# mindspore-lab/minddiffusion

Measured on AMD Instinct MI355X. Metric: 512x512 txt2img latents/sec (50-step DDIM), higher is better.
Workload: dtype f16; 1 GPU; SDv2 txt2img 512x512 (64x64 latent), 50-step DDIM, CFG 9.0, batch 1 per GPU (BASELINE.json configs[1]); synthetic seeded weights + synthetic text conditioning; global_batch=1, parallelism=batch-shard x1, hip_graph=True, rccl_world_size=1, broadcast_bytes=0, ddim_steps=50, unet_batch_per_gpu=2, sampler=ddim, cfg_dup_prefix=False

## Files before the change

minddiffusion_amd/_lib.py:

```python
import ctypes
import os

_HERE = os.path.dirname(os.path.abspath(__file__))
LIB_PATH = os.environ.get("MDX_LIBRARY") or os.path.join(_HERE, "libmdx.so")

c_void_p = ctypes.c_void_p
c_int = ctypes.c_int
c_uint = ctypes.c_uint
c_long = ctypes.c_long
c_float = ctypes.c_float
c_size_t = ctypes.c_size_t


class MdxError(RuntimeError):
    pass


class GemmDesc(ctypes.Structure):
    _fields_ = [
        ("a", c_void_p), ("a2", c_void_p), ("c1", c_int), ("c2", c_int),
        ("w", c_void_p), ("bias", c_void_p), ("rowbias", c_void_p), ("rowbias_ld", c_int),
        ("residual", c_void_p), ("residual_ld", c_int),
        ("out", c_void_p), ("out_ld", c_int),
        ("B", c_int), ("H", c_int), ("W", c_int), ("N", c_int),
# ... 136 lines not shown
                                       c_int, c_int, c_int, c_void_p]),
    "mdx_mask_feather_f32": (c_int, [c_void_p, c_void_p, c_int, c_void_p, c_int, c_int, c_int, c_void_p]),
    "mdx_inpaint_composite_f32": (c_int, [c_void_p, c_void_p, c_void_p, c_int, c_void_p, c_void_p, c_int, c_int, c_int,
                                          c_int, c_void_p]),
    "mdx_philox_u32": (c_int, [c_void_p, c_uint, c_uint, c_void_p, c_int, c_long, c_void_p]),
    "mdx_randn_f32": (c_int, [c_void_p, c_uint, c_uint, c_float, c_float, c_void_p, c_int, c_long, c_void_p]),
    "mdx_randn_slots_f32": (c_int, [c_void_p, c_uint, c_uint, c_float, c_float, c_void_p, c_void_p, c_void_p, c_int, c_int,
                                    c_long, c_void_p]),
    "mdx_slot_blend_f32": (c_int, [c_void_p, c_void_p, c_void_p, c_void_p, c_uint, c_uint, c_void_p, c_void_p, c_void_p,
                                   c_void_p, c_int, c_int, c_int, c_int, c_int, c_void_p]),
    "mdx_softmax_rows_f16": (c_int, [c_void_p, c_long, c_int, c_int, c_float, c_void_p]),
    "mdx_probe_mfma_32x32x16_f16": (c_int, [c_void_p, c_void_p, c_void_p, c_void_p]),
    "mdx_probe_mfma_16x16x32_f16": (c_int, [c_void_p, c_void_p, c_void_p, c_void_p]),
    "mdx_probe_gemm_trace": (c_int, [c_void_p, c_size_t]),
    "mdx_probe_valu_rate": (c_int, [c_int, c_int, c_int, c_void_p, c_void_p]),
    "mdx_probe_mix_rate": (c_int, [c_int, c_int, c_int, c_void_p, c_void_p]),
    "mdx_probe_l2_stream": (c_int, [c_void_p, c_size_t, ctypes.c_uint, c_int, c_int, c_int, c_int, c_void_p, c_void_p]),
    "mdx_probe_dma_stream": (c_int, [c_void_p, c_size_t, c_int, c_int, c_int, c_int, c_int, c_int, c_void_p, c_void_p]),
}

_lib = None
_ENV_OPTIONS = {
    "MDX_GEMM_TUNED": ("gemm_tuned", int), "MDX_GEMM_BM": ("gemm_bm", int), "MDX_GEMM_BN": ("gemm_bn", int),
    "MDX_GEMM_CFG": ("gemm_ring", lambda v: int(v.split(",")[-1])), "MDX_GEMM_HALO": ("gemm_halo", int),
    "MDX_GEMM_HALO8": ("gemm_halo8", int), "MDX_GEMM_SPLITK_FIXUP_MAX": ("gemm_splitk_fixup_max", int),
    "MDX_GEMM_SPREAD": ("gemm_spread", int), "MDX_HALO_NSB": ("halo_nsb", int), "MDX_GN_MIN_BLOCKS": ("gn_min_blocks", int),
    "MDX_GN_FUSED": ("gn_fused", int), "MDX_GN_COL_CHUNKS": ("gn_col_chunks", int),
    "MDX_GEMM_CONV8P": ("gemm_conv8p", int), "MDX_GEMM_CONV8P_MIN_M": ("gemm_conv8p_min_m", int),
    "MDX_GEMM_SUBPIXEL_MIN_TILES": ("gemm_subpixel_min_tiles", int), "MDX_GEMM_CONV8P_VAR": ("gemm_conv8p_var", int),
    "MDX_ATTN8": ("attn8", int), "MDX_ATTN8_MIN_BLOCKS": ("attn8_min_blocks", int),
    "MDX_GN_WIDE_ROWS": ("gn_wide_rows", int), "MDX_GN_BOOST_MB": ("gn_boost_mb", int), "MDX_ATTN_OCC3": ("attn_occ3", int), "MDX_ATTN_KV_SPLIT": ("attn_kv_split", int),
    "MDX_ATTN_FAST_STAGE": ("attn_fast_stage", int), "MDX_GN_PREFETCH": ("gn_prefetch", int), "MDX_GEMM_LN_PREFETCH": ("gemm_ln_prefetch", int),
    "MDX_GEMM_DENSE_ISSUE": ("gemm_dense_issue", int), "MDX_GEMM_LEAN_DENSE": ("gemm_lean_dense", int),
    "MDX_ATTN_PIPE": ("attn_pipe", int),
}


def load():
    global _lib
    if _lib is not None:
        return _lib
    if not os.path.exists(LIB_PATH):
        raise MdxError(
            f"{LIB_PATH} not found: the HIP extension is required (no CPU fallback). "
            "Build it with `python -c 'import __graft_entry__ as g; g.build()'` or `make -C minddiffusion_amd/csrc`.")
    import torch
    lib = ctypes.CDLL(LIB_PATH)
    for name, (res, args) in SIGNATURES.items():
        fn = getattr(lib, name)
        fn.restype = res
        fn.argtypes = args
    for env, (name, conv) in _ENV_OPTIONS.items():
        if env in os.environ:
            rc = lib.mdx_set_option(name.encode(), conv(os.environ[env]))
            if rc != 0:
                raise MdxError(f"{env}: {lib.mdx_last_error().decode()}")
    _lib = lib
    return lib


def check(rc, what):
    if rc != 0:
        msg = load().mdx_last_error()
        raise MdxError(f"{what} failed (rc={rc}): {msg.decode() if msg else ''}")
```

minddiffusion_amd/csrc/gemm.hip:

```cpp
#include "mdx_common.h"
#include "gemm_internal.h"

#include <algorithm>
#include <type_traits>

namespace {


template <int BM, int BN, int BK, int NS, bool SWAP, bool FASTK, int NW, bool GNA = false, bool EXT = false>
__global__ __launch_bounds__(NW * 64, NW == 4 ? 2 : 1) void gemm_kernel(const GemmParams p) {
    mdx_kernarg_touch<sizeof(GemmParams)>();
    constexpr int WROWS = BM / (NW / 2);
    constexpr int TM = WROWS / 32;
    constexpr int TN = BN / 64;
    static_assert(TM >= 1, "tile too short for this many waves");
    constexpr int ROWB = BK * 2;
    constexpr int CPRW = BK / 8;
    constexpr int RPI = 64 / CPRW;
    constexpr int RP256 = 256 / ROWB;
    constexpr int KS = BK / 16;
    constexpr int A_BYTES = BM * ROWB;
    constexpr int B_BYTES = BN * ROWB;
    constexpr int STAGE = A_BYTES + B_BYTES;
    constexpr int AJ = BM / RPI / NW;
    constexpr int BJ = BN / RPI / NW;
    static_assert(AJ >= 1 && BJ >= 1, "tile too small for this many loader waves");
    extern __shared__ __attribute__((aligned(16))) char smem[];

    const int tid = threadIdx.x;
    const int lane = tid & 63;
    const int wave = __builtin_amdgcn_readfirstlane(tid >> 6);
    const int wm = wave >> 1, wn = wave & 1;
    const int hi = lane >> 5;
    const int l31 = lane & 31;

    const int ntiles = p.tiles_m * p.tiles_n;
    const int tile_id = p.spread ? (int)(blockIdx.x % (unsigned)ntiles) : (blockIdx.x & 7) * p.tiles_per_xcd + (blockIdx.x >> 3);
// ... 291 lines not shown
            using I2 = std::integral_constant<int, 2>;
            using I3 = std::integral_constant<int, 3>;
            rdfrag(I0{}, 0); rdfrag(I1{}, 1); rdfrag(I2{}, 2); rdfrag(I3{}, 3);
            __builtin_amdgcn_sched_barrier(0);
            mfmas(I0{}); mfmas(I1{}); mfmas(I2{}); mfmas(I3{});
        } else {
            rdfrag(I0{}, 0);
            __builtin_amdgcn_sched_barrier(0);
#pragma unroll
            for (int ks = 0; ks < KS; ks += 2) {
                rdfrag(I1{}, ks + 1);
                __builtin_amdgcn_sched_barrier(0);
                mfmas(I0{});
                __builtin_amdgcn_sched_barrier(0);
                if (ks + 2 < KS) {
                    rdfrag(I0{}, ks + 2);
                    __builtin_amdgcn_sched_barrier(0);
                }
                mfmas(I1{});
                __builtin_amdgcn_sched_barrier(0);
            }
        }
        rd = (rd + 1 == NS) ? 0 : rd + 1;
        wr = (wr + 1 == NS) ? 0 : wr + 1;
    }

    __syncthreads();
    trace_mark(p, 3);
    if constexpr (SWAP) asm volatile("" ::"v"(touch_ln), "v"(touch_s));
    gemm_epilogue<BM, BN, SWAP, NW, LinearRows, 0, 0, EXT>(p, acc, smem, LinearRows{m0}, n0, split, bpre, tile_m, tile_id);
    trace_mark(p, 4);
}

template <int BM, int BN, int NSB, bool SWAP, int PW, bool BDIR = false, bool W4 = false>
__global__ __launch_bounds__(BM * 2, BM == 128 ? 2 : 1) void conv3x3_halo_kernel(const GemmParams p) {
    static_assert(PW == 16 || (PW == 8 && BM == 128), "patch width 16, or 8 with two-sample tiles");
    static_assert(!W4 || (BDIR && BM == 128 && BN == 128 && !SWAP), "W4: weight-streaming 128 x 128 tiles with slab output");
    constexpr int NW = BM / 32;
    constexpr int PH = BM / 16;
    constexpr int HWD = PW + 2;
    constexpr int WROWS = W4 ? BM : BM / (NW / 2);
    constexpr int TM = WROWS / 32;
    constexpr int TN = W4 ? 1 : BN / 64;
    constexpr int HROWS = PW == 16 ? (PH + 2) * 18 : (BM / 64) * 100;
    constexpr int HINST = (HROWS + 7) / 8;
    constexpr int HALO_BYTES = HINST * 1024;
    constexpr int HJ = (HINST + NW - 1) / NW;
    constexpr int B_BYTES = BN * 128;
    constexpr int BJ = BN / 8 / NW;
    static_assert(BJ >= 1, "weight tile too small for this many loader waves");
    extern __shared__ __attribute__((aligned(16))) char smem[];
    mdx_kernarg_touch<sizeof(GemmParams)>();

    const int tid = threadIdx.x;
    const int lane = tid & 63;
    const int wave = __builtin_amdgcn_readfirstlane(tid >> 6);
    const int wm = W4 ? 0 : wave >> 1, wn = W4 ? wave : wave & 1;
    const int hi = lane >> 5;
    const int l31 = lane & 31;

    const int ntiles = p.tiles_m * p.tiles_n;
    const int tile_id = p.spread ? (int)(blockIdx.x % (unsigned)ntiles) : (blockIdx.x & 7) * p.tiles_per_xcd + (blockIdx.x >> 3);
    if (tile_id >= ntiles) return;
    int tile_m, tile_n;
    if (p.n_fastest) {
        tile_m = tile_id / p.tiles_n;
        tile_n = tile_id - tile_m * p.tiles_n;
    } else {
        tile_n = tile_id / p.tiles_m;
        tile_m = tile_id - tile_n * p.tiles_m;
    }
    trace_mark(p, 0);
    const int n0 = tile_n * BN;
    const int pw = PW == 16 ? p.W >> 4 : 1, ph = PW == 16 ? p.H / PH : 1;
    const int pb = PW == 16 ? tile_m / (ph * pw) : tile_m * (BM / 64);
    const int prem = PW == 16 ? tile_m - pb * (ph * pw) : 0;
    const int py0 = (prem / pw) * PH, px0 = (prem % pw) * 16;
    const int split = p.spread ? (int)(blockIdx.x / (unsigned)ntiles) : (int)blockIdx.y;
    const int kt_begin = split * p.ktiles_per_split;
    const int kt_end = min(p.ktiles, kt_begin + p.ktiles_per_split);
    const int nt = kt_end - kt_begin;
    const int c_begin = kt_begin / 9, c_end = kt_end / 9;

    const __amdgpu_buffer_rsrc_t rs_a = make_rsrc(p.a, p.a_bytes);
    const __amdgpu_buffer_rsrc_t rs_w = make_rsrc(p.w, p.w_bytes);

    const int lrow = lane >> 3, lchk = lane & 7;
    unsigned hal_off[HJ];
    const unsigned row_bytes = (unsigned)p.cin * 2;
#pragma unroll
    for (int q = 0; q < HJ; ++q) {
        const int hp = (wave * HJ + q) * 8 + lrow;
        if constexpr (PW == 16) {
            const int hr = hp / 18, hc = hp - hr * 18;
            const int y = py0 - 1 + hr, x = px0 - 1 + hc;
            const bool ok = hp < HROWS && y >= 0 && y < p.H && x >= 0 && x < p.W;
            hal_off[q] = ok ? (unsigned)((pb * p.H + y) * p.W + x) * row_bytes + (unsigned)((lchk ^ ((hc >> 1) & 7)) * 16)
                            : MDX_OOB;
        } else {
            const int sm = hp / 100, r = hp - sm * 100;
            const int hr = r / 10, hc = r - hr * 10;
            const int y = hr - 1, x = hc - 1;
            const bool ok = hp < HROWS && pb + sm < p.B && y >= 0 && y < 8 && x >= 0 && x < 8;
            const int key = ((hc >> 1) & 3) | ((hr & 1) << 2);
            hal_off[q] = ok ? (unsigned)(((pb + sm) * 8 + y) * 8 + x) * row_bytes + (unsigned)((lchk ^ key) * 16) : MDX_OOB;
        }
    }
    unsigned b_off[BJ];
#pragma unroll
    for (int j = 0; j < BJ; ++j) {
        const int row = (wave * BJ + j) * 8 + lrow;
        const int panel = (n0 >> 6) + (row >> 6);
        b_off[j] = (unsigned)(((size_t)panel * p.kt64) * 8192 + ((row & 63) * 8 + lchk) * 16);
    }
    auto dma_halo = [&](int q, int chunk, int hb) {
        if (wave * HJ + q >= HINST) return;
        const unsigned off = hal_off[q] == MDX_OOB ? MDX_OOB : hal_off[q] + (unsigned)chunk * 128u;
        dma16(rs_a, smem + hb * HALO_BYTES + (wave * HJ + q) * 1024, off);
    };
    auto dma_b = [&](int kt, int stage) {
        char* sb = smem + 2 * HALO_BYTES + stage * B_BYTES;
#pragma unroll
        for (int j = 0; j < BJ; ++j) dma16s(rs_w, sb + (wave * BJ + j) * 1024, b_off[j], (unsigned)kt * 8192u);
    };

    f32x16 acc[TM][TN];
#pragma unroll
    for (int i = 0; i < TM; ++i)
#pragma unroll
        for (int j = 0; j < TN; ++j)
#pragma unroll
            for (int r = 0; r < 16; ++r) acc[i][j][r] = 0.f;

    int hp0[TM];
#pragma unroll
    for (int i = 0; i < TM; ++i) {
        const int q = wm * WROWS + i * 32 + l31;
        hp0[i] = PW == 16 ? (q >> 4) * 18 + (q & 15) : (q >> 6) * 100 + ((q >> 3) & 7) * 10 + (q & 7);
    }
    const int swz_b = (l31 >> 1) & 7;
    const int b_row_off = 2 * HALO_BYTES + (wn * (BN / 2) + l31) * 128;

    float bpre[16];
    gemm_bias_prefetch<BN, SWAP, NW>(p, n0, bpre);

    if constexpr (BDIR) {
        constexpr int PFB = 12;
        const unsigned kpieces = (unsigned)p.kt64 * 4u;
        unsigned pbase[TN];
#pragma unroll
        for (int j = 0; j < TN; ++j)
            pbase[j] = (unsigned)((n0 + (W4 ? wn * 32 : wn * (BN / 2) + j * 32)) >> 5) * kpieces + (unsigned)kt_begin * 4u;
        const unsigned voffw = (unsigned)lane * 16u;
#pragma unroll
        for (int q = 0; q < HJ; ++q) dma_halo(q, c_begin, 0);
        u32x4 ring[TN][PFB];
#pragma unroll
        for (int q = 0; q < PFB; ++q)
#pragma unroll
            for (int j = 0; j < TN; ++j) ring[j][q] = __builtin_amdgcn_raw_buffer_load_b128(rs_w, voffw, (pbase[j] + q) * 1024u, 0);
        trace_mark(p, 1);
        unsigned step = 0;
        for (int c = c_begin; c < c_end; ++c) {
            const int hb = (c - c_begin) & 1;
            asm volatile("s_waitcnt vmcnt(%0)" ::"n"(PFB * TN) : "memory");
            __builtin_amdgcn_s_barrier();
            if (c + 1 < c_end) {
#pragma unroll
                for (int q = 0; q < HJ; ++q) dma_halo(q, c + 1, hb ^ 1);
            }
#pragma unroll
            for (int tap = 0; tap < 9; ++tap) {
                const int ky = tap / 3, kx = tap - ky * 3;
                const int dq = ky * HWD + kx;
                int a_row[TM], a_key[TM];
#pragma unroll
                for (int i = 0; i < TM; ++i) {
                    a_row[i] = hb * HALO_BYTES + (hp0[i] + dq) * 128;
                    if constexpr (PW == 16)
                        a_key[i] = ((((l31 & 15) + kx) >> 1) & 7) << 4;
                    else
                        a_key[i] = (((((l31 & 7) + kx) >> 1) & 3) | ((((l31 >> 3) + ky) & 1) << 2)) << 4;
                }
#pragma unroll
                for (int s = 0; s < 4; ++s) {
                    f16x8 af[TM];
#pragma unroll
                    for (int i = 0; i < TM; ++i)
                        af[i] = *reinterpret_cast<const f16x8*>(smem + a_row[i] + (((2 * s + hi) << 4) ^ a_key[i]));
                    constexpr int dummy = 0;
                    (void)dummy;
                    const int rp = (tap * 4 + s) % PFB;
#pragma unroll
                    for (int j = 0; j < TN; ++j) {
                        const f16x8 b = __builtin_bit_cast(f16x8, ring[j][rp]);
                        ring[j][rp] = __builtin_amdgcn_raw_buffer_load_b128(rs_w, voffw, (pbase[j] + step + (unsigned)(tap * 4 + s) + PFB) * 1024u, 0);
#pragma unroll
                        for (int i = 0; i < TM; ++i) {
                            if constexpr (SWAP)
                                acc[i][j] = __builtin_amdgcn_mfma_f32_32x32x16_f16(b, af[i], acc[i][j], 0, 0, 0);
                            else
                                acc[i][j] = __builtin_amdgcn_mfma_f32_32x32x16_f16(af[i], b, acc[i][j], 0, 0, 0);
                        }
                    }
                    __builtin_amdgcn_sched_barrier(0);
                }
            }
            step += 36;
        }
        asm volatile("s_waitcnt vmcnt(0)" ::: "memory");
        __syncthreads();
        trace_mark(p, 3);
        if constexpr (W4) {
            float* wsz = p.ws + (size_t)split * p.M * p.N;
            const int n = n0 + wn * 32 + l31;
#pragma unroll
            for (int i = 0; i < TM; ++i)
#pragma unroll
                for (int r = 0; r < 16; ++r) {
                    const int row = i * 32 + (r & 3) + 8 * (r >> 2) + 4 * hi;
                    int m;
                    if constexpr (PW == 16)
                        m = (pb * p.H + py0) * p.W + px0 + (row >> 4) * p.W + (row & 15);
                    else
                        m = tile_m * BM + row;
                    if (m < p.M && n < p.N) wsz[(size_t)m * p.N + n] = acc[i][0][r];
                }
            trace_mark(p, 4);
            return;
        } else {
            if constexpr (PW == 16)
                gemm_epilogue<BM, BN, SWAP, NW, PatchRows, 0, 2>(p, acc, smem, PatchRows{(pb * p.H + py0) * p.W + px0, p.W, pb}, n0,
                                                                          split, bpre, tile_m, tile_id);
            else
                gemm_epilogue<BM, BN, SWAP, NW>(p, acc, smem, LinearRows{tile_m * BM}, n0, split, bpre, tile_m, tile_id);
            trace_mark(p, 4);
            return;
        }
    }
    if constexpr (!BDIR) {
    float2* gn_tab = reinterpret_cast<float2*>(smem + 2 * HALO_BYTES + NSB * B_BYTES);
    if constexpr (PW == 16) {
        if (p.gn_cs) {
            float2* csum = reinterpret_cast<float2*>(smem);
            const int cpg = p.cin >> 5;
// ... 470 lines not shown
void launch_cfg(const GemmParams& p, bool swap, bool fastk, dim3 grid, hipStream_t st) {
    if (swap) {
        if (fastk)
            launch_one<BM, BN, BK, NS, true, true, NW>(p, grid, st);
        else
            launch_one<BM, BN, BK, NS, true, false, NW>(p, grid, st);
    } else {
        if (fastk)
            launch_one<BM, BN, BK, NS, false, true, NW>(p, grid, st);
        else
            launch_one<BM, BN, BK, NS, false, false, NW>(p, grid, st);
    }
}

template <int BM, int BN>
bool launch_bn(const GemmParams& p, int ns, bool swap, bool fastk, dim3 grid, hipStream_t st, bool nw8 = false) {
    if constexpr (BM == 128) {
        if (nw8 && (ns == 2 || ns == 3)) {
            if (ns == 2) launch_cfg<128, BN, 64, 2, 8>(p, swap, fastk, grid, st); else launch_cfg<128, BN, 64, 3, 8>(p, swap, fastk, grid, st);
            return true;
        }
    }
    if (ns == 2) launch_cfg<BM, BN, 64, 2, 4>(p, swap, fastk, grid, st);
    else if (ns == 3) launch_cfg<BM, BN, 64, 3, 4>(p, swap, fastk, grid, st);
    else if (BM == 128 && ns == 4) launch_cfg<128, BN, 64, 4, 4>(p, swap, fastk, grid, st);
    else if (BM == 128 && ns == 5) launch_cfg<128, BN, 64, 5, 4>(p, swap, fastk, grid, st);
    else if (BM == 64 && ns == 4) launch_cfg<64, BN, 64, 4, 4>(p, swap, fastk, grid, st);
    else if (BM == 64 && ns == 5) launch_cfg<64, BN, 64, 5, 4>(p, swap, fastk, grid, st);
    else if (BM == 64 && ns == 6) launch_cfg<64, BN, 64, 6, 4>(p, swap, fastk, grid, st);
    else return false;
    return true;
}

template <int BM, int BN, int NSB, bool SWAP, int PW = 16, bool BDIR = false, bool W4 = false>
void launch_halo(const GemmParams& p, dim3 grid, hipStream_t st) {
    constexpr size_t hinst = ((PW == 16 ? (BM / 16 + 2) * 18 : (BM / 64) * 100) + 7) / 8;
    constexpr size_t ring = 2 * hinst * 1024 + (BDIR ? 0 : (size_t)NSB * BN * 128);
    constexpr size_t epi = (size_t)BM * (BN + 8) * 2 + 4096;
    constexpr size_t lds0 = ring > epi ? ring : epi;
    constexpr size_t gn_tab_max = (BDIR || PW != 16) ? 0 : 640 * 8;
    const size_t lds = lds0 + (p.gn_cs ? (size_t)p.cin * 8 : 0);
    static MdxPerDeviceOnce attr_once;
    if (attr_once.first()) {
        (void)hipFuncSetAttribute(reinterpret_cast<const void*>(&conv3x3_halo_kernel<BM, BN, NSB, SWAP, PW, BDIR, W4>),
                                  hipFuncAttributeMaxDynamicSharedMemorySize, (int)(lds0 + gn_tab_max));
    }
    hipLaunchKernelGGL((conv3x3_halo_kernel<BM, BN, NSB, SWAP, PW, BDIR, W4>), grid, dim3(BM * 2), lds, st, p);
}

template <int BN, int PW>
void launch_halo_bdir(const GemmParams& p, bool swap, dim3 grid, hipStream_t st) {
    if (swap) launch_halo<128, BN, 2, true, PW, true>(p, grid, st); else launch_halo<128, BN, 2, false, PW, true>(p, grid, st);
}
template <int PW>
void launch_halo_bdir_w4(const GemmParams& p, dim3 grid, hipStream_t st) {
    launch_halo<128, 128, 2, false, PW, true, true>(p, grid, st);
}

template <int BM, int BN, int PW = 16>
void launch_halo_cfg(const GemmParams& p, int nsb, bool swap, dim3 grid, hipStream_t st) {
    if (nsb == 4) {
        if (swap) launch_halo<BM, BN, 4, true, PW>(p, grid, st); else launch_halo<BM, BN, 4, false, PW>(p, grid, st);
    } else if (nsb == 3) {
        if (swap) launch_halo<BM, BN, 3, true, PW>(p, grid, st); else launch_halo<BM, BN, 3, false, PW>(p, grid, st);
    } else {
        if (swap) launch_halo<BM, BN, 2, true, PW>(p, grid, st); else launch_halo<BM, BN, 2, false, PW>(p, grid, st);
    }
}

}

int mdx_gemm_launch_plan(const GemmParams& p, const GemmPlan& pl, hipStream_t st) {
    const dim3 grid = pl.grid;
    const bool swap = pl.swap, wide = pl.bn == 128;
    int rc;
    switch (pl.form) {
        case GEMM_CONV8P:
            rc = mdx_conv8p_launch(p, pl.bn, st);
            if (rc != MDX_OK) return rc;
            MDX_LAUNCH_CHECK("mdx_gemm_f16(conv8p)");
            return MDX_OK;
        case GEMM_LEAN:
        case GEMM_LEAN_XA:
            rc = mdx_dense_launch(p, pl, st);
            if (rc != MDX_OK) return rc;
            break;
        case GEMM_HALO:
            if (pl.bm == 256) {
                if (wide) launch_halo_cfg<256, 128>(p, pl.ring, swap, grid, st); else launch_halo_cfg<256, 64>(p, pl.ring, swap, grid, st);
            } else if (pl.pw == 8) {
                if (wide) launch_halo_cfg<128, 128, 8>(p, pl.ring, swap, grid, st); else launch_halo_cfg<128, 64, 8>(p, pl.ring, swap, grid, st);
            } else {
                if (wide) launch_halo_cfg<128, 128>(p, pl.ring, swap, grid, st); else launch_halo_cfg<128, 64>(p, pl.ring, swap, grid, st);
            }
            break;
        case GEMM_HALO_FRAG:
            if (pl.pw == 8) {
                if (wide) launch_halo_bdir<128, 8>(p, swap, grid, st); else launch_halo_bdir<64, 8>(p, swap, grid, st);
            } else {
                if (wide) launch_halo_bdir<128, 16>(p, swap, grid, st); else launch_halo_bdir<64, 16>(p, swap, grid, st);
            }
            break;
        case GEMM_HALO_FRAG_W4:
            if (pl.pw == 8) launch_halo_bdir_w4<8>(p, grid, st); else launch_halo_bdir_w4<16>(p, grid, st);
            break;
        case GEMM_GNA:
            if (pl.bm == 64) {
                if (wide) launch_gna<64, 128>(p, pl.ring, swap, grid, st); else launch_gna<64, 64>(p, pl.ring, swap, grid, st);
            } else {
                if (wide) launch_gna<128, 128>(p, pl.ring, swap, grid, st); else launch_gna<128, 64>(p, pl.ring, swap, grid, st);
            }
            break;
        case GEMM_EXT:
            if (pl.bm == 64) {
                if (wide) launch_ext<64, 128>(p, pl.ring, swap, grid, st); else launch_ext<64, 64>(p, pl.ring, swap, grid, st);
            } else {
                if (wide) launch_ext<128, 128>(p, pl.ring, swap, grid, st); else launch_ext<128, 64>(p, pl.ring, swap, grid, st);
            }
            break;
        case GEMM_GENERIC:
        case GEMM_GENERIC_NW8: {
            const bool nw8 = pl.form == GEMM_GENERIC_NW8;
            bool ok;
            if (pl.bm == 64)
                ok = wide ? launch_bn<64, 128>(p, pl.ring, swap, pl.fastk, grid, st) : launch_bn<64, 64>(p, pl.ring, swap, pl.fastk, grid, st);
            else
                ok = wide ? launch_bn<128, 128>(p, pl.ring, swap, pl.fastk, grid, st, nw8) : launch_bn<128, 64>(p, pl.ring, swap, pl.fastk, grid, st, nw8);
            MDX_REQUIRE(ok, "mdx_gemm_f16: internal error: the plan names a generic tile %d x %d at ring depth %d that is not built", pl.bm,
                        pl.bn, pl.ring);
            break;
        }
    }
    MDX_LAUNCH_CHECK("mdx_gemm_f16");
    if (pl.reduce == GEMM_REDUCE_NONE || pl.reduce == GEMM_REDUCE_DEFERRED) return MDX_OK;
    if (pl.reduce == GEMM_REDUCE_COLSTATS) {
// ... 14 lines not shown
```

minddiffusion_amd/csrc/gemm_internal.h:

```cpp
#pragma once
#include "mdx_common.h"

namespace mdx_int {

struct GemmParams {
    const f16* a;
    const f16* a2;
    const f16* w;
    const float* bias;
    const float* rowbias;
    const f16* residual;
    f16* out;
    f16* out2;
    float* ws;
    unsigned* tickets;
    int c1, c2, cin;
    int rowbias_ld, residual_ld, out_ld, out2_ld, n_split;
    float* stats_out;
    float* colstats_out;
    const float* ln_stats;
    const float* ln_s;
    int ln_nt;
    int bn_hint;
    int st_hint;
// ... 38 lines not shown
};

}
using mdx_int::GemmParams;

enum GemmForm {
    GEMM_GENERIC,
    GEMM_GENERIC_NW8,
    GEMM_GNA,
    GEMM_EXT,
    GEMM_LEAN,
    GEMM_LEAN_XA,
    GEMM_HALO,
    GEMM_HALO_FRAG,
    GEMM_HALO_FRAG_W4,
    GEMM_CONV8P
};
enum GemmReduce { GEMM_REDUCE_NONE, GEMM_REDUCE_PLAIN, GEMM_REDUCE_EXT, GEMM_REDUCE_COLSTATS, GEMM_REDUCE_DEFERRED };
struct TunedEntry;
struct GemmPlan {
    GemmForm form;
    int bm, bn;
    int ring;
    int pw;
    int nsplit;
    bool fixup;
    bool swap, fastk;
    dim3 grid;
    const TunedEntry* tuned;
    int colstats_rows;
    GemmReduce reduce;
    size_t ws_head, ws_per_split;
};
int mdx_gemm_launch_plan(const GemmParams& p, const GemmPlan& pl, hipStream_t st);

bool mdx_dense_takes_desc(const GemmParams& p, int bn);
bool mdx_dense_takes(const GemmParams& p, int bm, int bn, int ring, int nsplit, bool fixup, bool nw8);
int mdx_dense_launch(const GemmParams& p, const GemmPlan& pl, hipStream_t st);
bool mdx_conv8p_eligible(const GemmParams& p);
int mdx_conv8p_pick_bn(const GemmParams& p, int bn_hint);
int mdx_conv8p_tiles(const GemmParams& p);
size_t mdx_conv8p_plan(GemmParams& p, int bn, size_t workspace_bytes, bool have_workspace, bool query_only);
int mdx_conv8p_launch(const GemmParams& p, int bn, hipStream_t st);

namespace {


__device__ __forceinline__ f16x4 cvt4(float a, float b, float c, float d) {
    f16x4 v;
    v[0] = (f16)a;
    v[1] = (f16)b;
    v[2] = (f16)c;
    v[3] = (f16)d;
    return v;
}

struct Row8Extras {
    float4 r0, r1;
    f16x8 res;
};

__device__ __forceinline__ Row8Extras epilogue_prefetch_row8(const GemmParams& p, int m, int n) {
    Row8Extras x;
    if (p.rowbias) {
        const int b = m / p.HoWo;
        const float4* rb = reinterpret_cast<const float4*>(p.rowbias + (size_t)b * p.rowbias_ld + n);
// ... 633 lines not shown
```

minddiffusion_amd/csrc/gemm_plan.hip:

```cpp
#include "mdx_common.h"
#include "gemm_internal.h"

#include <stdlib.h>

#include <algorithm>
#include <map>
#include <mutex>
#include <utility>
#include <vector>

static int fill_params(const mdx_gemm_desc* d, GemmParams& p) {
    MDX_REQUIRE(d && d->a && d->w && d->out, "mdx_gemm_f16: null pointer");
    MDX_REQUIRE(d->ksize == 1 || d->ksize == 3, "mdx_gemm_f16: ksize must be 1 or 3 (got %d)", d->ksize);
    MDX_REQUIRE(d->stride == 1 || d->stride == 2, "mdx_gemm_f16: stride must be 1 or 2");
    MDX_REQUIRE(!(d->upsample && d->stride != 1), "mdx_gemm_f16: upsample requires stride 1");
    MDX_REQUIRE(d->B > 0 && d->H > 0 && d->W > 0 && d->N > 0, "mdx_gemm_f16: bad extents");
    MDX_REQUIRE(d->c1 > 0 && d->c1 % 8 == 0 && d->c2 >= 0 && d->c2 % 8 == 0, "mdx_gemm_f16: c1/c2 must be multiples of 8");
    MDX_REQUIRE((d->c2 == 0) == (d->a2 == nullptr), "mdx_gemm_f16: a2/c2 mismatch");
    MDX_REQUIRE(d->N % 8 == 0, "mdx_gemm_f16: N must be a multiple of 8 (got %d)", d->N);
    p.a = (const f16*)d->a;
    p.a2 = (const f16*)d->a2;
    p.w = (const f16*)d->w;
    p.bias = d->bias;
    p.rowbias = d->rowbias;
// ... 418 lines not shown
    pl.fastk = (p.cin % 64 == 0) && (p.c2 == 0 || p.c1 % 64 == 0);
    MDX_REQUIRE(pl.fastk || p.c2 == 0, "mdx_gemm_f16: two-source input needs c1 %% 64 == 0 and Cin %% 64 == 0");
    const int ntiles = p.tiles_m * p.tiles_n;
    p.tiles_per_xcd = (ntiles + 7) / 8;
    p.inv_tiles_n = p.tiles_n > 1 ? (unsigned)((0x100000000ull + (unsigned)p.tiles_n - 1) / (unsigned)p.tiles_n) : 0u;
    p.inv_tiles_m = p.tiles_m > 1 ? (unsigned)((0x100000000ull + (unsigned)p.tiles_m - 1) / (unsigned)p.tiles_m) : 0u;
    p.res_bytes = p.residual ? (unsigned)std::min<size_t>((size_t)p.M * (size_t)p.residual_ld * 2, 0x7fffffffull) : 0u;
    p.n_fastest = ((size_t)p.M * p.cin >= (size_t)p.N * p.K) ? 1 : 0;
    p.spread = (p.tiles_m == 1 && mdx_opt(MDX_OPT_GEMM_SPREAD)) ? 1 : 0;
    pl.grid = p.spread ? dim3(ntiles * ns, 1) : dim3(8 * p.tiles_per_xcd, ns);
    const bool nw8 = stages >= 10;
    const int st_req = nw8 ? stages - 8 : stages;
    const int optring = mdx_opt(MDX_OPT_GEMM_RING);
    int ring = optring;
    if (!(optring >= 2 && optring <= 5)) {
        ring = (ntiles * ns <= 256 || bm + bn <= 192) ? 3 : 2;
        if (st_req >= 2 && st_req <= 6) ring = st_req;
    }
    pl.swap = (ns == 1 || pl.fixup) && (p.out_mode == MDX_OUT_ROWMAJOR);
    const bool lean = !halo && mdx_dense_takes(p, bm, bn, ring, ns, pl.fixup, nw8);
    MDX_REQUIRE(bn != 160 || lean, "mdx_gemm_f16: the 128 x 160 tile exists in the lean dense kernel only (ring depth 2 | 3, four waves; got stages %d)",
                stages);

    MDX_REQUIRE(!d->defer_reduce || ns > 1, "mdx_gemm_f16: defer_reduce set but the launch does not split K");
    MDX_REQUIRE(!p.xa_k || (lean && bn == 64 && ns == 1 && (p.HoWo % bm) == 0),
                "mdx_gemm_f16: the cross-attention epilogue needs the lean dense kernel on %d x 64 tiles inside one sample (got tile %d x %d, %d splits)",
                bm, bm, bn, ns);
    MDX_REQUIRE(!d->w_frag || halo, "mdx_gemm_f16: fragment-major weights (w_frag) are read by the HALO 3x3 conv only");

    if (halo) {
        if (d->w_frag) {
            MDX_REQUIRE(bm == 128, "mdx_gemm_f16: fragment-major weights run on 128-row HALO tiles only (got tile_m %d)", bm);
            pl.form = (bn == 128 && ns > 1 && !pl.fixup) ? GEMM_HALO_FRAG_W4 : GEMM_HALO_FRAG;
        } else {
            pl.form = GEMM_HALO;
            pl.ring = (bm == 256 || bn == 64) ? 3 : 2;
            if (st_req >= 2 && st_req <= 4) pl.ring = st_req;
            if (mdx_opt(MDX_OPT_HALO_NSB) >= 2 && mdx_opt(MDX_OPT_HALO_NSB) <= 4) pl.ring = mdx_opt(MDX_OPT_HALO_NSB);
        }
    } else if (p.gn_cs || p.epilogue == MDX_EPI_PRELU || p.d2s_c) {
        pl.form = p.gn_cs ? GEMM_GNA : GEMM_EXT;
        pl.ring = ring >= 3 ? 3 : 2;
    } else if (lean) {
        pl.form = p.xa_k ? GEMM_LEAN_XA : GEMM_LEAN;
        pl.ring = ring;
    } else {
        pl.form = (nw8 && bm == 128 && (ring == 2 || ring == 3)) ? GEMM_GENERIC_NW8 : GEMM_GENERIC;
        pl.ring = ring;
        MDX_REQUIRE(ring <= (bm == 128 ? 5 : 6), "mdx_gemm_f16: unsupported tile configuration bk=%d ns=%d", 64,
                    (optring >= 2 && optring <= 5) ? optring : 2);
    }
    return MDX_OK;
}

static unsigned long long* g_gemm_trace = nullptr;
static size_t g_gemm_trace_slots = 0;

extern "C" int mdx_probe_gemm_trace(void* buf, size_t bytes) {
    g_gemm_trace = (unsigned long long*)buf;
    g_gemm_trace_slots = buf ? bytes / 64 : 0;
    return MDX_OK;
}

struct TicketPools {
    std::mutex mu;
    std::map<std::pair<int, const void*>, unsigned*> slot;
// ... 292 lines not shown
```

minddiffusion_amd/csrc/mdx_common.h:

```cpp
#pragma once
#include <hip/hip_runtime.h>
#include <stdarg.h>
#include <stdio.h>

#include "mdx.h"

typedef _Float16 f16;
typedef f16 f16x2 __attribute__((ext_vector_type(2)));
typedef f16 f16x4 __attribute__((ext_vector_type(4)));
typedef f16 f16x8 __attribute__((ext_vector_type(8)));
typedef float f32x4 __attribute__((ext_vector_type(4)));
typedef float f32x16 __attribute__((ext_vector_type(16)));

#define MDX_LDS_PTR(p) ((__attribute__((address_space(3))) void*)(p))

void mdx_set_error(const char* fmt, ...);

#define MDX_REQUIRE(cond, ...)            \
    do {                                  \
        if (!(cond)) {                    \
            mdx_set_error(__VA_ARGS__);   \
            return MDX_E_INVALID;         \
        }                                 \
    } while (0)
// ... 19 lines not shown
};
int mdx_internal_split_info(const mdx_gemm_desc* d, MdxSplitInfo* info);

enum MdxOpt {
    MDX_OPT_GEMM_TUNED,
    MDX_OPT_GEMM_BM,
    MDX_OPT_GEMM_BN,
    MDX_OPT_GEMM_RING,
    MDX_OPT_GEMM_HALO,
    MDX_OPT_GEMM_HALO8,
    MDX_OPT_GEMM_SPLITK_FIXUP_MAX,
    MDX_OPT_GEMM_SPREAD,
    MDX_OPT_HALO_NSB,
    MDX_OPT_GN_MIN_BLOCKS,
    MDX_OPT_GN_FUSED,
    MDX_OPT_GN_COL_CHUNKS,
    MDX_OPT_GEMM_CONV8P,
    MDX_OPT_GEMM_CONV8P_MIN_M,
    MDX_OPT_GEMM_SUBPIXEL_MIN_TILES,
    MDX_OPT_GEMM_CONV8P_VAR,
    MDX_OPT_ATTN8,
    MDX_OPT_ATTN8_MIN_BLOCKS,
    MDX_OPT_GN_WIDE_ROWS,
    MDX_OPT_GN_FUSED_SMALL,
    MDX_OPT_GN_BOOST_MB,
    MDX_OPT_ATTN_OCC3,
    MDX_OPT_ATTN_KV_SPLIT,
    MDX_OPT_ATTN_FAST_STAGE,
    MDX_OPT_GN_PREFETCH,
    MDX_OPT_GEMM_DENSE_ISSUE,
    MDX_OPT_GEMM_LN_PREFETCH,
    MDX_OPT_GEMM_LEAN_DENSE,
    MDX_OPT_ATTN_PIPE,
    MDX_OPT_COUNT
};
int mdx_opt(int id);

struct MdxPerDeviceOnce {
    bool done[64] = {};
    bool first() {
        int dv = 0;
        if (hipGetDevice(&dv) != hipSuccess || dv < 0 || dv >= 64) return true;
        if (done[dv]) return false;
        done[dv] = true;
        return true;
    }
};

__device__ __forceinline__ float sigmoid_fast(float x) {
    return __builtin_amdgcn_rcpf(1.0f + __builtin_amdgcn_exp2f(-1.4426950408889634f * x));
}

__device__ __forceinline__ float silu_f(float x) { return x * sigmoid_fast(x); }

__device__ __forceinline__ float quick_gelu_f(float x) { return x * sigmoid_fast(1.702f * x); }

__device__ __forceinline__ float gelu_tanh_f(float x) {
    const float u = 0.7978845608028654f * (x + 0.044715f * x * x * x);
    return x * sigmoid_fast(2.0f * u);
}

__device__ __forceinline__ float wave_sum(float v) {
#pragma unroll
    for (int o = 32; o > 0; o >>= 1) v += __shfl_xor(v, o, 64);
    return v;
}
// ... 36 lines not shown
```

minddiffusion_amd/csrc/small.hip:

```cpp
#include "mdx_common.h"

#include <string.h>

static thread_local char g_err[512] = "";

void mdx_set_error(const char* fmt, ...) {
    va_list ap;
    va_start(ap, fmt);
    vsnprintf(g_err, sizeof(g_err), fmt, ap);
    va_end(ap);
}

extern "C" const char* mdx_last_error(void) { return g_err; }

static const char* const g_opt_names[MDX_OPT_COUNT] = {"gemm_tuned", "gemm_bm", "gemm_bn", "gemm_ring", "gemm_halo", "gemm_halo8",
                                                        "gemm_splitk_fixup_max", "gemm_spread", "halo_nsb", "gn_min_blocks",
                                                        "gn_fused", "gn_col_chunks", "gemm_conv8p", "gemm_conv8p_min_m", "gemm_subpixel_min_tiles", "gemm_conv8p_var", "attn8", "attn8_min_blocks",
                                                        "gn_wide_rows", "gn_fused_small", "gn_boost_mb", "attn_occ3", "attn_kv_split", "attn_fast_stage",
                                                        "gn_prefetch", "gemm_dense_issue", "gemm_ln_prefetch", "gemm_lean_dense", "attn_pipe"};
static int g_opt[MDX_OPT_COUNT] = {1, 0, 0, 0, 1, 1, 4, 1, 0, 512, 1, 4, 1, 4096, 32, 0, 0, 192, 0, 0, 40, 1, 1, 1, 1, 1, 1, 1, 1};

int mdx_opt(int id) { return g_opt[id]; }

extern "C" int mdx_set_option(const char* name, int value) {
    MDX_REQUIRE(name, "mdx_set_option: null name");
    for (int i = 0; i < MDX_OPT_COUNT; ++i)
        if (!strcmp(name, g_opt_names[i])) {
            g_opt[i] = value;
            return MDX_OK;
        }
    mdx_set_error("mdx_set_option: unknown option '%s'", name);
    return MDX_E_INVALID;
}

extern "C" int mdx_get_option(const char* name, int* value) {
    MDX_REQUIRE(name && value, "mdx_get_option: null argument");
    for (int i = 0; i < MDX_OPT_COUNT; ++i)
        if (!strcmp(name, g_opt_names[i])) {
            *value = g_opt[i];
            return MDX_OK;
        }
    mdx_set_error("mdx_get_option: unknown option '%s'", name);
    return MDX_E_INVALID;
}
extern "C" int mdx_version(void) { return 1; }

namespace {

__global__ __launch_bounds__(256) void nchw_to_nhwc_kernel(const float* __restrict__ x, f16* __restrict__ y, int B,
                                                           int C, int HW, int Cpad) {
    const size_t total = (size_t)B * HW * Cpad;
    for (size_t i = (size_t)blockIdx.x * 256 + threadIdx.x; i < total; i += (size_t)gridDim.x * 256) {
        const int c = (int)(i % Cpad);
// ... 985 lines not shown
```

Baseline: 5.566 latents/s.

## Deepen weight-streaming ring in halo conv and double-buffer A fragment reads

The fragment-major halo conv kernel now issues its initial weight-ring loads before the halo setup, and lets 64-column tiles use ring depths of 18 or 36, picked through a new option, a stages field or a tuned entry. The K loop is fully unrolled into 36 compile-time steps, and the LDS A-fragment reads are double-buffered so the next step's reads overlap the current MFMAs. With depth 36, the bias prefetch moves after the main loop to save registers. The default depth stays 12, so the main default change is the earlier prefetch plus the restructured unrolled loop, which adds register pressure.

```diff
diff --git a/minddiffusion_amd/_lib.py b/minddiffusion_amd/_lib.py
--- a/minddiffusion_amd/_lib.py
+++ b/minddiffusion_amd/_lib.py
@@ -192,7 +192,7 @@
     "MDX_GN_WIDE_ROWS": ("gn_wide_rows", int), "MDX_GN_BOOST_MB": ("gn_boost_mb", int), "MDX_ATTN_OCC3": ("attn_occ3", int), "MDX_ATTN_KV_SPLIT": ("attn_kv_split", int),
     "MDX_ATTN_FAST_STAGE": ("attn_fast_stage", int), "MDX_GN_PREFETCH": ("gn_prefetch", int), "MDX_GEMM_LN_PREFETCH": ("gemm_ln_prefetch", int),
     "MDX_GEMM_DENSE_ISSUE": ("gemm_dense_issue", int), "MDX_GEMM_LEAN_DENSE": ("gemm_lean_dense", int),
-    "MDX_ATTN_PIPE": ("attn_pipe", int),
+    "MDX_ATTN_PIPE": ("attn_pipe", int), "MDX_HALO_STREAM_RING": ("halo_stream_ring", int),
 }
 
 
diff --git a/minddiffusion_amd/csrc/gemm.hip b/minddiffusion_amd/csrc/gemm.hip
--- a/minddiffusion_amd/csrc/gemm.hip
+++ b/minddiffusion_amd/csrc/gemm.hip
@@ -3,6 +3,7 @@
 
 #include <algorithm>
 #include <type_traits>
+#include <utility>
 
 namespace {
 
@@ -360,10 +361,22 @@
     trace_mark(p, 4);
 }
 
-template <int BM, int BN, int NSB, bool SWAP, int PW, bool BDIR = false, bool W4 = false>
+template <int V>
+using IC = std::integral_constant<int, V>;
+template <int N, class F, int... I>
+__device__ __forceinline__ void static_for_seq(F&& f, std::integer_sequence<int, I...>) {
+    (f(IC<I>{}), ...);
+}
+template <int N, class F>
+__device__ __forceinline__ void static_for(F&& f) {
+    static_for_seq<N>(f, std::make_integer_sequence<int, N>{});
+}
+
+template <int BM, int BN, int NSB, bool SWAP, int PW, bool BDIR = false, bool W4 = false, int PFB = 12>
 __global__ __launch_bounds__(BM * 2, BM == 128 ? 2 : 1) void conv3x3_halo_kernel(const GemmParams p) {
     static_assert(PW == 16 || (PW == 8 && BM == 128), "patch width 16, or 8 with two-sample tiles");
     static_assert(!W4 || (BDIR && BM == 128 && BN == 128 && !SWAP), "W4: weight-streaming 128 x 128 tiles with slab output");
+    static_assert(PFB == 12 || (BDIR && !W4 && (PFB == 18 || PFB == 36)), "ring depths 18 | 36: the 2 x 2 weight-streaming form only");
     constexpr int NW = BM / 32;
     constexpr int PH = BM / 16;
     constexpr int HWD = PW + 2;
@@ -413,6 +426,22 @@
     const __amdgpu_buffer_rsrc_t rs_a = make_rsrc(p.a, p.a_bytes);
     const __amdgpu_buffer_rsrc_t rs_w = make_rsrc(p.w, p.w_bytes);
 
+    [[maybe_unused]] u32x4 ring[BDIR ? TN : 1][BDIR ? PFB : 1];
+    [[maybe_unused]] unsigned pbase[TN];
+    [[maybe_unused]] const unsigned voffw = (unsigned)(threadIdx.x & 63) * 16u;
+    if constexpr (BDIR) {
+        const unsigned kpieces = (unsigned)p.kt64 * 4u;
+        const int wn_ = W4 ? wave : wave & 1;
+#pragma unroll
+        for (int j = 0; j < TN; ++j)
+            pbase[j] = (unsigned)((n0 + (W4 ? wn_ * 32 : wn_ * (BN / 2) + j * 32)) >> 5) * kpieces + (unsigned)kt_begin * 4u;
+#pragma unroll
+        for (int q = 0; q < PFB; ++q)
+#pragma unroll
+            for (int j = 0; j < TN; ++j) ring[j][q] = __builtin_amdgcn_raw_buffer_load_b128(rs_w, voffw, (pbase[j] + q) * 1024u, 0);
+        __builtin_amdgcn_sched_barrier(0);
+    }
+
     const int lrow = lane >> 3, lchk = lane & 7;
     unsigned hal_off[HJ];
     const unsigned row_bytes = (unsigned)p.cin * 2;
@@ -469,76 +498,73 @@
     const int swz_b = (l31 >> 1) & 7;
     const int b_row_off = 2 * HALO_BYTES + (wn * (BN / 2) + l31) * 128;
 
+    constexpr bool BIAS_LATE = BDIR && PFB == 36;
     float bpre[16];
-    gemm_bias_prefetch<BN, SWAP, NW>(p, n0, bpre);
+    if constexpr (!BIAS_LATE) gemm_bias_prefetch<BN, SWAP, NW>(p, n0, bpre);
 
     if constexpr (BDIR) {
-        constexpr int PFB = 12;
-        const unsigned kpieces = (unsigned)p.kt64 * 4u;
-        unsigned pbase[TN];
-#pragma unroll
-        for (int j = 0; j < TN; ++j)
-            pbase[j] = (unsigned)((n0 + (W4 ? wn * 32 : wn * (BN / 2) + j * 32)) >> 5) * kpieces + (unsigned)kt_begin * 4u;
-        const unsigned voffw = (unsigned)lane * 16u;
+        static_assert(36 % PFB == 0 && PFB * TN <= 63, "ring depth: a divisor of 36 whose loads the vmcnt field can count");
 #pragma unroll
         for (int q = 0; q < HJ; ++q) dma_halo(q, c_begin, 0);
-        u32x4 ring[TN][PFB];
-#pragma unroll
-        for (int q = 0; q < PFB; ++q)
-#pragma unroll
-            for (int j = 0; j < TN; ++j) ring[j][q] = __builtin_amdgcn_raw_buffer_load_b128(rs_w, voffw, (pbase[j] + q) * 1024u, 0);
         trace_mark(p, 1);
         unsigned step = 0;
         for (int c = c_begin; c < c_end; ++c) {
             const int hb = (c - c_begin) & 1;
-            asm volatile("s_waitcnt vmcnt(%0)" ::"n"(PFB * TN) : "memory");
+            if (c == c_begin)
+                asm volatile("s_waitcnt vmcnt(0)" ::: "memory");
+            else
+                asm volatile("s_waitcnt vmcnt(%0)" ::"n"(PFB * TN) : "memory");
             __builtin_amdgcn_s_barrier();
+            if (c == c_begin) trace_mark(p, 2);
             if (c + 1 < c_end) {
 #pragma unroll
                 for (int q = 0; q < HJ; ++q) dma_halo(q, c + 1, hb ^ 1);
             }
-#pragma unroll
-            for (int tap = 0; tap < 9; ++tap) {
-                const int ky = tap / 3, kx = tap - ky * 3;
-                const int dq = ky * HWD + kx;
-                int a_row[TM], a_key[TM];
+            f16x8 af[2][TM];
+            auto rd_a = [&](auto ks_c, auto slot_c) {
+                constexpr int ks = decltype(ks_c)::value, slot = decltype(slot_c)::value;
+                constexpr int tap = ks / 4, s = ks & 3;
+                constexpr int ky = tap / 3, kx = tap - ky * 3;
+                constexpr int dq = ky * HWD + kx;
 #pragma unroll
                 for (int i = 0; i < TM; ++i) {
-                    a_row[i] = hb * HALO_BYTES + (hp0[i] + dq) * 128;
+                    const int a_row = hb * HALO_BYTES + (hp0[i] + dq) * 128;
+                    int a_key;
                     if constexpr (PW == 16)
-                        a_key[i] = ((((l31 & 15) + kx) >> 1) & 7) << 4;
+                        a_key = ((((l31 & 15) + kx) >> 1) & 7) << 4;
                     else
-                        a_key[i] = (((((l31 & 7) + kx) >> 1) & 3) | ((((l31 >> 3) + ky) & 1) << 2)) << 4;
-                }
-#pragma unroll
-                for (int s = 0; s < 4; ++s) {
-                    f16x8 af[TM];
-#pragma unroll
-                    for (int i = 0; i < TM; ++i)
-                        af[i] = *reinterpret_cast<const f16x8*>(smem + a_row[i] + (((2 * s + hi) << 4) ^ a_key[i]));
-                    constexpr int dummy = 0;
-                    (void)dummy;
-                    const int rp = (tap * 4 + s) % PFB;
-#pragma unroll
-                    for (int j = 0; j < TN; ++j) {
-                        const f16x8 b = __builtin_bit_cast(f16x8, ring[j][rp]);
-                        ring[j][rp] = __builtin_amdgcn_raw_buffer_load_b128(rs_w, voffw, (pbase[j] + step + (unsigned)(tap * 4 + s) + PFB) * 1024u, 0);
-#pragma unroll
-                        for (int i = 0; i < TM; ++i) {
-                            if constexpr (SWAP)
-                                acc[i][j] = __builtin_amdgcn_mfma_f32_32x32x16_f16(b, af[i], acc[i][j], 0, 0, 0);
-                            else
-                                acc[i][j] = __builtin_amdgcn_mfma_f32_32x32x16_f16(af[i], b, acc[i][j], 0, 0, 0);
-                        }
+                        a_key = (((((l31 & 7) + kx) >> 1) & 3) | ((((l31 >> 3) + ky) & 1) << 2)) << 4;
+                    af[slot][i] = *reinterpret_cast<const f16x8*>(smem + a_row + (((2 * s + hi) << 4) ^ a_key));
+                }
+            };
+            rd_a(IC<0>{}, IC<0>{});
+            __builtin_amdgcn_sched_barrier(0);
+            auto kstep = [&](auto ks_c) {
+                constexpr int ks = decltype(ks_c)::value;
+                constexpr int cur = ks & 1;
+                if constexpr (ks + 1 < 36) rd_a(IC<ks + 1>{}, IC<cur ^ 1>{});
+                constexpr int rp = ks % PFB;
+#pragma unroll
+                for (int j = 0; j < TN; ++j) {
+                    const f16x8 b = __builtin_bit_cast(f16x8, ring[j][rp]);
+                    ring[j][rp] = __builtin_amdgcn_raw_buffer_load_b128(rs_w, voffw, (pbase[j] + step + (unsigned)(ks + PFB)) * 1024u, 0);
+#pragma unroll
+                    for (int i = 0; i < TM; ++i) {
+                        if constexpr (SWAP)
+                            acc[i][j] = __builtin_amdgcn_mfma_f32_32x32x16_f16(b, af[cur][i], acc[i][j], 0, 0, 0);
+                        else
+                            acc[i][j] = __builtin_amdgcn_mfma_f32_32x32x16_f16(af[cur][i], b, acc[i][j], 0, 0, 0);
                     }
-                    __builtin_amdgcn_sched_barrier(0);
-                }
-            }
+                }
+                __builtin_amdgcn_sched_barrier(0);
+            };
+            static_for<36>(kstep);
             step += 36;
         }
         asm volatile("s_waitcnt vmcnt(0)" ::: "memory");
         __syncthreads();
         trace_mark(p, 3);
+        if constexpr (BIAS_LATE) gemm_bias_prefetch<BN, SWAP, NW>(p, n0, bpre);
         if constexpr (W4) {
             float* wsz = p.ws + (size_t)split * p.M * p.N;
             const int n = n0 + wn * 32 + l31;
@@ -1075,7 +1101,7 @@
     return true;
 }
 
-template <int BM, int BN, int NSB, bool SWAP, int PW = 16, bool BDIR = false, bool W4 = false>
+template <int BM, int BN, int NSB, bool SWAP, int PW = 16, bool BDIR = false, bool W4 = false, int PFB = 12>
 void launch_halo(const GemmParams& p, dim3 grid, hipStream_t st) {
     constexpr size_t hinst = ((PW == 16 ? (BM / 16 + 2) * 18 : (BM / 64) * 100) + 7) / 8;
     constexpr size_t ring = 2 * hinst * 1024 + (BDIR ? 0 : (size_t)NSB * BN * 128);
@@ -1085,15 +1111,26 @@
     const size_t lds = lds0 + (p.gn_cs ? (size_t)p.cin * 8 : 0);
     static MdxPerDeviceOnce attr_once;
     if (attr_once.first()) {
-        (void)hipFuncSetAttribute(reinterpret_cast<const void*>(&conv3x3_halo_kernel<BM, BN, NSB, SWAP, PW, BDIR, W4>),
+        (void)hipFuncSetAttribute(reinterpret_cast<const void*>(&conv3x3_halo_kernel<BM, BN, NSB, SWAP, PW, BDIR, W4, PFB>),
                                   hipFuncAttributeMaxDynamicSharedMemorySize, (int)(lds0 + gn_tab_max));
     }
-    hipLaunchKernelGGL((conv3x3_halo_kernel<BM, BN, NSB, SWAP, PW, BDIR, W4>), grid, dim3(BM * 2), lds, st, p);
-}
-
+    hipLaunchKernelGGL((conv3x3_halo_kernel<BM, BN, NSB, SWAP, PW, BDIR, W4, PFB>), grid, dim3(BM * 2), lds, st, p);
+}
+
+template <int BN, int PW, int PFB>
+void launch_halo_bdir_d(const GemmParams& p, bool swap, dim3 grid, hipStream_t st) {
+    if (swap) launch_halo<128, BN, 2, true, PW, true, false, PFB>(p, grid, st);
+    else launch_halo<128, BN, 2, false, PW, true, false, PFB>(p, grid, st);
+}
 template <int BN, int PW>
-void launch_halo_bdir(const GemmParams& p, bool swap, dim3 grid, hipStream_t st) {
-    if (swap) launch_halo<128, BN, 2, true, PW, true>(p, grid, st); else launch_halo<128, BN, 2, false, PW, true>(p, grid, st);
+bool launch_halo_bdir(const GemmParams& p, int depth, bool swap, dim3 grid, hipStream_t st) {
+    if (depth == 12) launch_halo_bdir_d<BN, PW, 12>(p, swap, grid, st);
+    else if constexpr (BN == 64) {
+        if (depth == 18) launch_halo_bdir_d<BN, PW, 18>(p, swap, grid, st);
+        else if (depth == 36) launch_halo_bdir_d<BN, PW, 36>(p, swap, grid, st);
+        else return false;
+    } else return false;
+    return true;
 }
 template <int PW>
 void launch_halo_bdir_w4(const GemmParams& p, dim3 grid, hipStream_t st) {
@@ -1138,12 +1175,16 @@
             }
             break;
         case GEMM_HALO_FRAG:
-            if (pl.pw == 8) {
-                if (wide) launch_halo_bdir<128, 8>(p, swap, grid, st); else launch_halo_bdir<64, 8>(p, swap, grid, st);
-            } else {
-                if (wide) launch_halo_bdir<128, 16>(p, swap, grid, st); else launch_halo_bdir<64, 16>(p, swap, grid, st);
-            }
+        {
+            bool ok;
+            if (pl.pw == 8)
+                ok = wide ? launch_halo_bdir<128, 8>(p, pl.ring, swap, grid, st) : launch_halo_bdir<64, 8>(p, pl.ring, swap, grid, st);
+            else
+                ok = wide ? launch_halo_bdir<128, 16>(p, pl.ring, swap, grid, st) : launch_halo_bdir<64, 16>(p, pl.ring, swap, grid, st);
+            MDX_REQUIRE(ok, "mdx_gemm_f16: internal error: the plan names a weight-streaming ring of %d pieces on %d-column tiles that is not built",
+                        pl.ring, pl.bn);
             break;
+        }
         case GEMM_HALO_FRAG_W4:
             if (pl.pw == 8) launch_halo_bdir_w4<8>(p, grid, st); else launch_halo_bdir_w4<16>(p, grid, st);
             break;
diff --git a/minddiffusion_amd/csrc/gemm_internal.h b/minddiffusion_amd/csrc/gemm_internal.h
--- a/minddiffusion_amd/csrc/gemm_internal.h
+++ b/minddiffusion_amd/csrc/gemm_internal.h
@@ -94,6 +94,8 @@
     GemmReduce reduce;
     size_t ws_head, ws_per_split;
 };
+inline bool mdx_halo_stream_depth_built(int bn, int depth) { return depth == 12 || (bn == 64 && (depth == 18 || depth == 36)); }
+constexpr int HALO_STREAM_RING_DEFAULT = 12;
 int mdx_gemm_launch_plan(const GemmParams& p, const GemmPlan& pl, hipStream_t st);
 
 bool mdx_dense_takes_desc(const GemmParams& p, int bn);
diff --git a/minddiffusion_amd/csrc/gemm_plan.hip b/minddiffusion_amd/csrc/gemm_plan.hip
--- a/minddiffusion_amd/csrc/gemm_plan.hip
+++ b/minddiffusion_amd/csrc/gemm_plan.hip
@@ -474,6 +474,29 @@
         if (d->w_frag) {
             MDX_REQUIRE(bm == 128, "mdx_gemm_f16: fragment-major weights run on 128-row HALO tiles only (got tile_m %d)", bm);
             pl.form = (bn == 128 && ns > 1 && !pl.fixup) ? GEMM_HALO_FRAG_W4 : GEMM_HALO_FRAG;
+            const int optd = mdx_opt(MDX_OPT_HALO_STREAM_RING);
+            const int cap = bn == 64 ? 36 : 12;
+            int depth = HALO_STREAM_RING_DEFAULT;
+            if (pl.form == GEMM_HALO_FRAG_W4) {
+                depth = 12;
+                MDX_REQUIRE(d->stages == 0 || d->stages == 12,
+                            "mdx_gemm_f16: the side-by-side weight-streaming form (128-column tiles, slab split-K) is built with a ring "
+                            "of 12 pieces only (got stages %d)", d->stages);
+            } else if (d->stages != 0) {
+                depth = d->stages;
+                MDX_REQUIRE(mdx_halo_stream_depth_built(bn, depth),
+                            "mdx_gemm_f16: weight-streaming ring depth (stages) %d is not built for %d-column tiles: 12%s", depth, bn,
+                            bn == 64 ? " | 18 | 36" : " only");
+            } else if (optd != 0) {
+                MDX_REQUIRE(mdx_halo_stream_depth_built(64, optd), "mdx_gemm_f16: option halo_stream_ring must be 0 | 12 | 18 | 36 (got %d)", optd);
+                depth = std::min(optd, cap);
+            } else if (pl.tuned && mdx_halo_stream_depth_built(64, pl.tuned->st)) {
+                depth = std::min(pl.tuned->st, cap);
+            }
+            pl.ring = depth;
+            MDX_REQUIRE(((unsigned long long)p.tiles_n * (bn / 32) * ((unsigned long long)p.kt64 * 4) + (unsigned long long)depth) * 1024ull <=
+                            0xffffffffull,
+                        "mdx_gemm_f16: fragment-major weights of this size cannot be addressed through a 32-bit piece offset");
         } else {
             pl.form = GEMM_HALO;
             pl.ring = (bm == 256 || bn == 64) ? 3 : 2;
diff --git a/minddiffusion_amd/csrc/mdx_common.h b/minddiffusion_amd/csrc/mdx_common.h
--- a/minddiffusion_amd/csrc/mdx_common.h
+++ b/minddiffusion_amd/csrc/mdx_common.h
@@ -75,6 +75,7 @@
     MDX_OPT_GEMM_LN_PREFETCH,
     MDX_OPT_GEMM_LEAN_DENSE,
     MDX_OPT_ATTN_PIPE,
+    MDX_OPT_HALO_STREAM_RING,
     MDX_OPT_COUNT
 };
 int mdx_opt(int id);
diff --git a/minddiffusion_amd/csrc/small.hip b/minddiffusion_amd/csrc/small.hip
--- a/minddiffusion_amd/csrc/small.hip
+++ b/minddiffusion_amd/csrc/small.hip
@@ -17,8 +17,8 @@
                                                         "gemm_splitk_fixup_max", "gemm_spread", "halo_nsb", "gn_min_blocks",
                                                         "gn_fused", "gn_col_chunks", "gemm_conv8p", "gemm_conv8p_min_m", "gemm_subpixel_min_tiles", "gemm_conv8p_var", "attn8", "attn8_min_blocks",
                                                         "gn_wide_rows", "gn_fused_small", "gn_boost_mb", "attn_occ3", "attn_kv_split", "attn_fast_stage",
-                                                        "gn_prefetch", "gemm_dense_issue", "gemm_ln_prefetch", "gemm_lean_dense", "attn_pipe"};
-static int g_opt[MDX_OPT_COUNT] = {1, 0, 0, 0, 1, 1, 4, 1, 0, 512, 1, 4, 1, 4096, 32, 0, 0, 192, 0, 0, 40, 1, 1, 1, 1, 1, 1, 1, 1};
+                                                        "gn_prefetch", "gemm_dense_issue", "gemm_ln_prefetch", "gemm_lean_dense", "attn_pipe", "halo_stream_ring"};
+static int g_opt[MDX_OPT_COUNT] = {1, 0, 0, 0, 1, 1, 4, 1, 0, 512, 1, 4, 1, 4096, 32, 0, 0, 192, 0, 0, 40, 1, 1, 1, 1, 1, 1, 1, 1, 0};
 
 int mdx_opt(int id) { return g_opt[id]; }
 
```

Result: no change. 5.568 latents/s, median of 2 (+0.0%).
